# JADGardner/neusky

Measured on AMD Instinct MI355X. Metric: train rays/sec on NeRF-OSR lk2 @1024 rays x 96 samples, higher is better.
Workload: dtype f32 in memory; forward products: fp16 hi + residual split, 3 x v_mfma_f32_32x32x16_f16 per product on power-of-two pre-scaled operands, one fp32 accumulator (~2^-22): FiLM-SIREN chains and the SDF / albedo field alike; backward products: the same fp16 split on per-row / per-matrix pre-scaled gradien; 1 GPU; full NeuSky train step (BASELINE configs[2]): 1024 rays/GPU x 96 samples, proposal 256+96, 512 illumination directions (256 upper-hemisphere DDF queries/ray), illumination decoder = this project's FiLM-SIREN H = 128 (RENI-shaped: latent 100x3; the reference's configured Attention decoder is absent from its tree), hash L16 F2 T2^19 x2, 256-wide MLPs; fwd + losses + bwd + all-reduce + 5 Adam groups; rays_per_gpu=1024, samples_per_ray=96, illumination_directions=512, parallelism=ray-sharded dp1, launcher=self-spawned, launch=HIP graph replay (1 graph/step + all-reduce + 5 Adam launches)

## Files before the change

include/neusky_hip.h:

```cpp
#ifndef NEUSKY_HIP_H
#define NEUSKY_HIP_H

#include <stdint.h>

#ifdef __cplusplus
extern "C" {
#endif

typedef void* nsky_stream_t;

const char* nsky_last_error(void);
int nsky_abi_version(void);

enum {
  NSKY_EPI_NONE = 0,
  NSKY_EPI_RELU = 1,
  NSKY_EPI_LEAKY = 2,
  NSKY_EPI_SIGMOID = 3,
  NSKY_EPI_SOFTPLUS = 4,
  NSKY_EPI_FILM = 5,
  NSKY_EPI_MUL_AUX = 6,
  NSKY_EPI_BWD_RELU = 7,
  NSKY_EPI_BWD_LEAKY = 8,
  NSKY_EPI_BWD_FILM = 9,
// ... 44 lines not shown
  const float* mo_w; const float* mo_b; int32_t mo_ld;
  const float* film_w[NSKY_FILM_MAX_LAYERS]; const float* film_b[NSKY_FILM_MAX_LAYERS]; int32_t film_ld[NSKY_FILM_MAX_LAYERS];
  const float* out_w; const float* out_b; int32_t out_ld;
} nsky_film_net;
int nsky_film_stream_layout(const nsky_film_net* net, int32_t direction, int64_t* stream_bytes, int32_t* n_tiles);
int nsky_film_pack(const nsky_film_net* net, int32_t direction, void* stream_buf, float* table, nsky_stream_t stream);
int nsky_film_chain_fwd(const nsky_film_net* net, const void* stream_buf, const float* table, const float* cond,
                        int32_t ldcond, const float* x, int32_t ldx, int32_t M, float* const* h_save, float* const* z_save,
                        float* const* y_save, float* res, int32_t ldres, nsky_stream_t stream);
int nsky_film_chain_bwd_film(const nsky_film_net* net, const void* stream_buf, const float* table, int32_t M, const float* d_res,
                             int32_t ldres, const float* h_last, const float* const* z_save, float* const* dz_save, float* dfp,
                             float* dfp_rowmax, float* gmax, float* d_x, int32_t ldx, nsky_stream_t stream);
int nsky_film_chain_bwd_map(const nsky_film_net* net, const void* stream_buf, const float* table, int32_t M, const float* dfp,
                            const float* dfp_rowmax, const float* const* h_save, float* const* dpre_save, float* d_cond,
                            int32_t ldcond, float* gmax, nsky_stream_t stream);
typedef struct {
  int32_t in_dim, hidden;
  const float* w0; int32_t ld0; const float* b0;
  const float* w1; int32_t ld1; const float* b1;
  const float* w2; const float* b2;
  float beta;
} nsky_sdf_net;
int nsky_sdf_stream_layout(const nsky_sdf_net* net, int32_t direction, int64_t* stream_bytes, int32_t* n_tiles);
int nsky_sdf_pack(const nsky_sdf_net* net, int32_t direction, void* stream_buf, float* table, nsky_stream_t stream);
int nsky_sdf_chain_fwd(const nsky_sdf_net* net, const void* stream_buf, const float* table, const float* E, int32_t ldE, int32_t M,
                       float* a0_save, float* a1_save, float* sdf, nsky_stream_t stream);
int nsky_sdf_chain_bwd(const nsky_sdf_net* net, const void* stream_buf, const float* table, int32_t M, const float* g_sdf,
                       const float* a0_save, const float* a1_save, float* dz1, float* dz0, float* dE, int32_t ldE, float* dw2,
                       float* db2, float* gmax, nsky_stream_t stream);

// ... 346 lines not shown
```

neusky_amd/csrc/film_chain.hip:

```cpp
#include "chain.h"

namespace {

constexpr int FWD_FRAG_BUFFERS = 3;


struct Layout {
  int NT, Gc, Gx, Gh;
  long base_map, base_film0, base_film, base_head, total_groups;
  int n_tiles;
};

__host__ __device__ inline Layout fwd_layout(const nsky_film_net& n) {
  Layout L;
  L.NT = n.hidden / 32;
  L.Gc = groups_of(n.cond_dim);
  L.Gx = groups_of(n.x_dim);
  L.Gh = groups_of(n.hidden);
  L.base_map = (long)L.NT * L.Gc;
  L.base_film0 = L.base_map + (long)(n.n_map - 1) * L.NT * L.Gh;
  L.base_film = L.base_film0 + (long)L.NT * (2 * L.Gh + L.Gx);
  L.base_head = L.base_film + (long)(n.n_film - 1) * L.NT * 3 * L.Gh;
  L.total_groups = L.base_head + L.Gh;
  L.n_tiles = n.n_map * L.NT + n.n_film * L.NT * 3 + 1;
// ... 125 lines not shown
}



struct FwdArgs {
  nsky_film_net net;
  const unsigned char* stream;
  const float* table;
  const float* cond; int ldcond;
  const float* x; int ldx;
  int M;
  float* h_save[MAXL];
  float* z_save[MAXL];
  float* y_save[MAXL];
  float* res; int ldres;
};


template <int H, int KSC, bool KEEP_Y = true>
__global__ __launch_bounds__(256, 1) void film_fwd_kernel(const FwdArgs a) {
  constexpr int NT = H / 32, KS = H / 16;
  __shared__ __attribute__((aligned(16))) unsigned char smem[RING_BYTES + (BIAS_FLOATS + SCALE_FLOATS) * 4];
  float* bl = reinterpret_cast<float*>(smem + RING_BYTES);
  const nsky_film_net& net = a.net;
  const int tid = threadIdx.x, lane = tid & 63;
  const int wave = __builtin_amdgcn_readfirstlane(tid >> 6);
  const int c = lane & 31, h = lane >> 5;
  float* sl = bl + BIAS_FLOATS;
  NSKY_STAGE_TABLE((BIAS_FLOATS + SCALE_FLOATS) / 4, 256, a.table, bl, tid);
  __syncthreads();
  WStream ws;
  ws_open<4, false, RING_GROUPS, true>(ws, a.stream, smem, wave, lane);

  const long rt = (long)blockIdx.x * 4 + wave;
// ... 7 lines not shown
  f16x8 hh[KS], hl[KS];
  float h_inv;
  {
    f16x8 ch[KSC], cl[KSC];
    const int ksc = ksteps_of(net.cond_dim);
    const float c_inv = load_planes<KSC>(a.cond + rowc * a.ldcond, (net.cond_dim + 3) & ~3, ksc, h, ch, cl);
    float hn[NT][16];
    float m = 0.0f;
#pragma unroll
    for (int t = 0; t < NT; ++t) {
      f32x16 acc;
#pragma unroll
      for (int r = 0; r < 16; ++r) acc[r] = 0.0f;
      product_dyn<KSC>(ws, ksc, ch, cl, acc);
      const float inv = c_inv * sl[tile++];
#pragma unroll
      for (int g = 0; g < 4; ++g) {
        const float4 b = *reinterpret_cast<const float4*>(bl + 32 * t + 8 * g + 4 * h);
        const float bb[4] = {b.x, b.y, b.z, b.w};
#pragma unroll
        for (int q = 0; q < 4; ++q) {
          const float v = fmaf(acc[4 * g + q], inv, bb[q]);
          const float o = v > 0.0f ? v : 0.2f * v;
          hn[t][4 * g + q] = o;
          m = fmaxf(m, fabsf(o));
        }
      }
      if (a.h_save[0] && wave_live) store_tile_nt(a.h_save[0] + (rt * NT + t) * 1024, lane, hn[t]);
    }
    const float s = row_scale(m, h_inv);
#pragma unroll
    for (int t = 0; t < NT; ++t)
#pragma unroll
      for (int u = 0; u < 2; ++u) {
        float x8[8];
#pragma unroll
        for (int j = 0; j < 8; ++j) x8[j] = hn[t][8 * u + j] * s;
        split8(x8, hh[2 * t + u], hl[2 * t + u]);
      }
  }
  for (int l = 1; l < n_map; ++l) {
    float hn[NT][16];
    float m = 0.0f;
    const float* bias = bl + l * H;
#pragma unroll
    for (int t = 0; t < NT; ++t) {
      f32x16 acc;
#pragma unroll
      for (int r = 0; r < 16; ++r) acc[r] = 0.0f;
      product<KS, 4, false, RING_GROUPS, FWD_FRAG_BUFFERS>(ws, hh, hl, acc);
      const float inv = h_inv * sl[tile++];
#pragma unroll
      for (int g = 0; g < 4; ++g) {
        const float4 b = *reinterpret_cast<const float4*>(bias + 32 * t + 8 * g + 4 * h);
        const float bb[4] = {b.x, b.y, b.z, b.w};
#pragma unroll
        for (int q = 0; q < 4; ++q) {
          const float v = fmaf(acc[4 * g + q], inv, bb[q]);
          const float o = v > 0.0f ? v : 0.2f * v;
          hn[t][4 * g + q] = o;
          m = fmaxf(m, fabsf(o));
        }
      }
      if (a.h_save[l] && wave_live) store_tile_nt(a.h_save[l] + (rt * NT + t) * 1024, lane, hn[t]);
    }
    const float s = row_scale(m, h_inv);
#pragma unroll
    for (int t = 0; t < NT; ++t)
#pragma unroll
      for (int u = 0; u < 2; ++u) {
        float x8[8];
#pragma unroll
        for (int j = 0; j < 8; ++j) x8[j] = hn[t][8 * u + j] * s;
        split8(x8, hh[2 * t + u], hl[2 * t + u]);
      }
  }
  f16x8 xh[1], xl[1];
  const float x_inv = load_planes<1>(a.x + rowc * a.ldx, (net.x_dim + 3) & ~3, 1, h, xh, xl);
  f16x8 yh[KS], yl[KS];
// ... 309 lines not shown
  ws_close();
}

struct BwdMapArgs {
  nsky_film_net net;
  const unsigned char* stream;
  const float* table;
  int M;
  const float* dfp;
  const float* dfp_rowmax;
  const float* h_save[MAXL];
  float* dpre_save[MAXL];
  float* d_cond; int ldcond;
  float* gmax;
  int full_wgs, tail_wgs, tail_k;
};

template <int H, bool ACTIVE, bool KEEP>
__device__ __forceinline__ void film_bwd_map_tile(const BwdMapArgs& a, WStream& ws, const float* sl, long rt, int lane) {
  constexpr int NT = H / 32, KS = H / 16, PW = 2;
  constexpr bool REGS = !KEEP && H <= 128;
  float dreg[REGS ? NT : 1][16];
  const nsky_film_net& net = a.net;
  const int c = lane & 31, h = lane >> 5;
  const long row = rt * 32 + c;
  const bool live = ACTIVE && row < a.M;
  const int nkb = 2 * net.n_film * H / 64, ntot = 2 * net.n_film * NT;
  float f_inv = 1.0f, f_scale = 1.0f;
  if (ACTIVE) f_scale = row_scale(a.dfp_rowmax[rt * 32 + c], f_inv);
  int tile = 0;
  const float* fblk = a.dfp + rt * ntot * 1024;
  const int top = net.n_map - 1;
  float m = 0.0f;
// ... 95 lines not shown
          float x8[8];
#pragma unroll
          for (int j = 0; j < 8; ++j) x8[j] = dv[8 * v + j] * s;
          split8(x8, ph[2 * u + v], pl[2 * u + v]);
        }
      }
      asm volatile("s_waitcnt vmcnt(0)" ::: "memory");
    }
    m = 0.0f;
    if (l > 0) {
      for (int u = 0; u < NT; ++u) {
        f32x16 acc;
        prod<KS, PW>(ws, ACTIVE, ph, pl, acc);
        if (ACTIVE) {
          const float inv = d_inv * sl[tile];
          float hv[16], dv[16];
          load_tile(a.h_save[l - 1] + (rt * NT + u) * 1024, lane, hv);
#pragma unroll
          for (int r = 0; r < 16; ++r) {
            const float g = acc[r] * inv;
            dv[r] = hv[r] > 0.0f ? g : 0.2f * g;
            m = fmaxf(m, fabsf(dv[r]));
          }
          if constexpr (REGS) {
#pragma unroll
            for (int uu = 0; uu < NT; ++uu)
              if (u == uu) {
#pragma unroll
                for (int r = 0; r < 16; ++r) dreg[uu][r] = dv[r];
              }
          } else {
            store_tile(a.dpre_save[l - 1] + (rt * NT + u) * 1024, lane, dv);
          }
          asm volatile("s_waitcnt vmcnt(0)" ::: "memory");
        }
        ++tile;
      }
// ... 5 lines not shown
        if (ACTIVE && a.d_cond && live) {
          const float inv = d_inv * sl[tile];
#pragma unroll
          for (int g = 0; g < 4; ++g) {
            const int fo = 32 * u + 8 * g + 4 * h;
            if (fo < a.ldcond)
              stg4(a.d_cond + row * a.ldcond + fo, make_float4(acc[4 * g] * inv, acc[4 * g + 1] * inv, acc[4 * g + 2] * inv, acc[4 * g + 3] * inv));
          }
        }
        ++tile;
      }
    }
  }
}

template <int H, bool KEEP = true>
__global__ __launch_bounds__(512, 2) void film_bwd_map_kernel(const BwdMapArgs a) {
  constexpr int PW = 2;
  __shared__ __attribute__((aligned(16))) unsigned char smem[RING_BYTES + SCALE_FLOATS * 4];
  float* sl = reinterpret_cast<float*>(smem + RING_BYTES);
  const int tid = threadIdx.x, lane = tid & 63;
  const int wave = __builtin_amdgcn_readfirstlane(tid >> 6);
  for (int i = tid; i < SCALE_FLOATS; i += 512) sl[i] = a.table[BIAS_FLOATS + i];
  __syncthreads();
  WStream ws;
  ws_open<PW>(ws, a.stream, smem, wave, lane);
  const long n_tiles = (a.M + 31) / 32;
  const long rt = tail_tile(a.full_wgs, a.tail_wgs, a.tail_k, n_tiles, wave);
  if (rt >= 0 && rt < n_tiles) film_bwd_map_tile<H, true, KEEP>(a, ws, sl, rt, lane);
  else film_bwd_map_tile<H, false, KEEP>(a, ws, sl, 0, lane);
  ws_close();
}

int check_net(const nsky_film_net* n, const char* who) {
  NSKY_CHECK_ARG(n, "%s: null network", who);
  NSKY_CHECK_ARG(n->hidden == 128 || n->hidden == 256, "%s: hidden width %d (128 or 256)", who, n->hidden);
  NSKY_CHECK_ARG(n->n_map >= 1 && n->n_map <= MAXL && n->n_film >= 1 && n->n_film <= MAXL, "%s: layer counts %d / %d", who, n->n_map, n->n_film);
  NSKY_CHECK_ARG(n->cond_dim >= 1 && n->cond_dim <= PACK_KMAX && n->x_dim >= 1 && n->x_dim <= 16 && n->out_dim >= 1 && n->out_dim <= 4,
                 "%s: cond_dim %d (<= %d), x_dim %d (<= 16), out_dim %d (<= 4)", who, n->cond_dim, PACK_KMAX, n->x_dim, n->out_dim);
  const int nb = n->n_map * n->hidden + 3 * n->n_film * n->hidden + 32;
  NSKY_CHECK_ARG(nb <= BIAS_FLOATS, "%s: %d bias values exceed the LDS table (%d)", who, nb, BIAS_FLOATS);
  NSKY_CHECK_ARG(fwd_layout(*n).n_tiles <= SCALE_FLOATS, "%s: %d weight tiles exceed the LDS scale table (%d)", who, fwd_layout(*n).n_tiles, SCALE_FLOATS);
  for (int l = 0; l < n->n_map; ++l) NSKY_CHECK_ARG(n->map_w[l] && n->map_ld[l] >= (l == 0 ? n->cond_dim : n->hidden), "%s: mapping layer %d", who, l);
  for (int l = 0; l < n->n_film; ++l) NSKY_CHECK_ARG(n->film_w[l] && n->film_ld[l] >= (l == 0 ? n->x_dim : n->hidden), "%s: FiLM layer %d", who, l);
  NSKY_CHECK_ARG(n->mo_w && n->mo_ld >= n->hidden && n->out_w && n->out_ld >= n->hidden, "%s: head weights", who);
// ... 15 lines not shown
}

extern "C" int nsky_film_pack(const nsky_film_net* net, int32_t direction, void* stream_buf, float* table, nsky_stream_t stream) {
  if (int rc = check_net(net, "nsky_film_pack")) return rc;
  NSKY_CHECK_ARG(direction >= 0 && direction <= 2 && stream_buf && table && ((uintptr_t)stream_buf % 16) == 0 && ((uintptr_t)table % 16) == 0, "nsky_film_pack: bad arguments");
  long groups;
  int tiles;
  dir_layout(*net, direction, groups, tiles);
  NSKY_CHECK_ARG(tiles <= SCALE_FLOATS, "nsky_film_pack: %d weight tiles exceed the scale table (%d)", tiles, SCALE_FLOATS);
  if (direction != 0) NSKY_CHECK_ARG(net->hidden % 128 == 0, "nsky_film_pack: backward streams need hidden %% 128 == 0");
  hipLaunchKernelGGL(film_pack_kernel, dim3(tiles + 1), dim3(256), 0, (hipStream_t)stream, *net, direction, (unsigned char*)stream_buf, table);
  NSKY_CHECK_LAUNCH("nsky_film_pack");
  return NSKY_OK;
}

extern "C" int nsky_film_chain_fwd(const nsky_film_net* net, const void* stream_buf, const float* table, const float* cond,
                                   int32_t ldcond, const float* x, int32_t ldx, int32_t M, float* const* h_save, float* const* z_save,
                                   float* const* y_save, float* res, int32_t ldres, nsky_stream_t stream) {
  if (int rc = check_net(net, "nsky_film_chain_fwd")) return rc;
  NSKY_CHECK_ARG(stream_buf && table && cond && x && res && M > 0, "nsky_film_chain_fwd: null operand / empty batch");
  NSKY_CHECK_ARG(ldcond % 4 == 0 && ldcond >= ((net->cond_dim + 3) & ~3) && ldx % 4 == 0 && ldx >= ((net->x_dim + 3) & ~3) && ldres >= 4 && ldres % 4 == 0,
                 "nsky_film_chain_fwd: leading dimensions (cond %d, x %d, res %d) must be multiples of 4 covering the padded widths", ldcond, ldx, ldres);
  NSKY_CHECK_ARG(((uintptr_t)cond % 16) == 0 && ((uintptr_t)x % 16) == 0 && ((uintptr_t)res % 16) == 0 && ((uintptr_t)stream_buf % 16) == 0 && ((uintptr_t)table % 16) == 0,
                 "nsky_film_chain_fwd: operands must be 16-byte aligned");
  FwdArgs a;
  a.net = *net;
  a.stream = (const unsigned char*)stream_buf; a.table = table;
  a.cond = cond; a.ldcond = ldcond; a.x = x; a.ldx = ldx; a.M = M; a.res = res; a.ldres = ldres;
  for (int l = 0; l < MAXL; ++l) {
    a.h_save[l] = (h_save && l < net->n_map) ? h_save[l] : nullptr;
    a.z_save[l] = (z_save && l < net->n_film) ? z_save[l] : nullptr;
    a.y_save[l] = (y_save && l < net->n_film) ? y_save[l] : nullptr;
  }
  const bool keep_y = a.y_save[0] != nullptr;
  NSKY_CHECK_ARG(keep_y || net->hidden == 128, "nsky_film_chain_fwd: NULL y_save needs hidden 128 (hidden %d: pass two ping-pong buffers)", net->hidden);
  for (int l = 0; l < net->n_film; ++l)
    NSKY_CHECK_ARG((a.y_save[l] != nullptr) == keep_y && ((uintptr_t)a.y_save[l] % 16) == 0, "nsky_film_chain_fwd: y_save[%d] missing / unaligned", l);
  const dim3 grid(ceil_div(M, 128));
  const int ksc = ksteps_of(net->cond_dim);
#define NSKY_FILM_FWD(HH, KK, KEEP) hipLaunchKernelGGL((film_fwd_kernel<HH, KK, KEEP>), grid, dim3(256), 0, (hipStream_t)stream, a)
  if (net->hidden == 256) { if (ksc <= 4) NSKY_FILM_FWD(256, 4, true); else NSKY_FILM_FWD(256, 20, true); }
  else if (keep_y) { if (ksc <= 4) NSKY_FILM_FWD(128, 4, true); else NSKY_FILM_FWD(128, 20, true); }
  else { if (ksc <= 4) NSKY_FILM_FWD(128, 4, false); else NSKY_FILM_FWD(128, 20, false); }
#undef NSKY_FILM_FWD
  NSKY_CHECK_LAUNCH("nsky_film_chain_fwd");
  return NSKY_OK;
}


extern "C" int nsky_film_chain_bwd_film(const nsky_film_net* net, const void* stream_buf, const float* table, int32_t M, const float* d_res,
                                        int32_t ldres, const float* h_last, const float* const* z_save, float* const* dz_save, float* dfp,
                                        float* dfp_rowmax, float* gmax, float* d_x, int32_t ldx, nsky_stream_t stream) {
  if (int rc = check_net(net, "nsky_film_chain_bwd_film")) return rc;
  NSKY_CHECK_ARG(stream_buf && table && d_res && h_last && z_save && dfp && dfp_rowmax && gmax && M > 0, "nsky_film_chain_bwd_film: null operand / empty batch");
  NSKY_CHECK_ARG(ldres >= 4 && ldres % 4 == 0 && ((uintptr_t)d_res % 16) == 0 && ((uintptr_t)h_last % 16) == 0 && ((uintptr_t)dfp % 16) == 0 &&
                     ((uintptr_t)stream_buf % 16) == 0 && ((uintptr_t)table % 16) == 0, "nsky_film_chain_bwd_film: alignment / ldres");
  NSKY_CHECK_ARG(net->hidden % 128 == 0, "nsky_film_chain_bwd_film: hidden %% 128");
  BwdFilmArgs a;
  a.net = *net; a.stream = (const unsigned char*)stream_buf; a.table = table; a.M = M; a.d_res = d_res; a.ldres = ldres; a.h_last = h_last;
  a.dfp = dfp; a.dfp_rowmax = dfp_rowmax; a.gmax = gmax; a.d_x = d_x; a.ldx = ldx;
  if (d_x) NSKY_CHECK_ARG(ldx % 4 == 0 && ldx >= ((net->x_dim + 3) & ~3) && ldx <= 16 && ((uintptr_t)d_x % 16) == 0, "nsky_film_chain_bwd_film: d_x layout (ldx %d)", ldx);
// ... 2 lines not shown
    a.dz_save[l] = (dz_save && l < net->n_film) ? dz_save[l] : nullptr;
  }
  const bool keep = a.dz_save[0] != nullptr;
  for (int l = 0; l < net->n_film; ++l)
    NSKY_CHECK_ARG(a.z_save[l] && (a.dz_save[l] != nullptr) == keep && ((uintptr_t)a.z_save[l] % 16) == 0 && ((uintptr_t)a.dz_save[l] % 16) == 0, "nsky_film_chain_bwd_film: z_save / dz_save[%d]", l);
  a.full_wgs = a.tail_wgs = a.tail_k = 0;
  const dim3 grid(ceil_div(ceil_div(M, 32), 4));
#define NSKY_FILM_BWD4(HH, KEEP) hipLaunchKernelGGL((film_bwd4_kernel<HH, KEEP>), grid, dim3(256), 0, (hipStream_t)stream, a)
  if (net->hidden == 256) { if (keep) NSKY_FILM_BWD4(256, true); else NSKY_FILM_BWD4(256, false); }
  else { if (keep) NSKY_FILM_BWD4(128, true); else NSKY_FILM_BWD4(128, false); }
#undef NSKY_FILM_BWD4
  NSKY_CHECK_LAUNCH("nsky_film_chain_bwd_film");
  return NSKY_OK;
}

extern "C" int nsky_film_chain_bwd_map(const nsky_film_net* net, const void* stream_buf, const float* table, int32_t M, const float* dfp,
                                       const float* dfp_rowmax, const float* const* h_save, float* const* dpre_save, float* d_cond,
                                       int32_t ldcond, float* gmax, nsky_stream_t stream) {
  if (int rc = check_net(net, "nsky_film_chain_bwd_map")) return rc;
  NSKY_CHECK_ARG(stream_buf && table && dfp && dfp_rowmax && h_save && gmax && M > 0, "nsky_film_chain_bwd_map: null operand / empty batch");
  NSKY_CHECK_ARG(((uintptr_t)dfp % 16) == 0 && ((uintptr_t)stream_buf % 16) == 0 && ((uintptr_t)table % 16) == 0, "nsky_film_chain_bwd_map: alignment");
  if (d_cond) NSKY_CHECK_ARG(ldcond % 4 == 0 && ldcond >= ((net->cond_dim + 3) & ~3) && ((uintptr_t)d_cond % 16) == 0, "nsky_film_chain_bwd_map: d_cond layout");
  NSKY_CHECK_ARG(net->hidden % 128 == 0, "nsky_film_chain_bwd_map: hidden %% 128");
  BwdMapArgs a;
  a.net = *net; a.stream = (const unsigned char*)stream_buf; a.table = table; a.M = M; a.dfp = dfp; a.dfp_rowmax = dfp_rowmax;
  a.d_cond = d_cond; a.ldcond = ldcond; a.gmax = gmax;
  for (int l = 0; l < MAXL; ++l) {
    a.h_save[l] = l < net->n_map ? h_save[l] : nullptr;
    a.dpre_save[l] = (dpre_save && l < net->n_map) ? dpre_save[l] : nullptr;
  }
  const bool regs = a.dpre_save[0] == nullptr;
  const bool keep = !regs && !(net->n_map > 1 && a.dpre_save[1] == a.dpre_save[0]);
  NSKY_CHECK_ARG(!regs || net->hidden == 128, "nsky_film_chain_bwd_map: NULL dpre_save needs hidden 128 (hidden %d: pass one shared buffer)", net->hidden);
  for (int l = 0; l < net->n_map; ++l)
    NSKY_CHECK_ARG(a.h_save[l] && (a.dpre_save[l] == nullptr) == regs && (keep || a.dpre_save[l] == a.dpre_save[0]) && ((uintptr_t)a.h_save[l] % 16) == 0 &&
                       ((uintptr_t)a.dpre_save[l] % 16) == 0, "nsky_film_chain_bwd_map: h_save / dpre_save[%d]", l);
  const TailPlan tp = tail_plan(ceil_div(M, 32), device_cus());
  a.full_wgs = tp.full_wgs; a.tail_wgs = tp.tail_wgs; a.tail_k = tp.tail_k;
  const dim3 grid(tp.full_wgs + tp.tail_wgs);
#define NSKY_FILM_BWD_MAP(HH, KEEP) hipLaunchKernelGGL((film_bwd_map_kernel<HH, KEEP>), grid, dim3(512), 0, (hipStream_t)stream, a)
  if (net->hidden == 256) { if (keep) NSKY_FILM_BWD_MAP(256, true); else NSKY_FILM_BWD_MAP(256, false); }
  else { if (keep) NSKY_FILM_BWD_MAP(128, true); else NSKY_FILM_BWD_MAP(128, false); }
#undef NSKY_FILM_BWD_MAP
  NSKY_CHECK_LAUNCH("nsky_film_chain_bwd_map");
  return NSKY_OK;
}
```

neusky_amd/hip.py:

```python
from __future__ import annotations

import ctypes as C
import os

import torch

_HERE = os.path.dirname(os.path.abspath(__file__))
LIB_PATH = os.path.join(_HERE, "libneusky_hip.so")


class NeuSkyHipError(RuntimeError):
    pass


if not os.path.exists(LIB_PATH):
    raise ImportError(
        f"{LIB_PATH} not found: build the HIP extension first (python -c 'import __graft_entry__ as g; g.build()'). "
        "neusky_amd has no CPU/PyTorch fallback."
    )
_lib = C.CDLL(LIB_PATH)

EPI_NONE, EPI_RELU, EPI_LEAKY, EPI_SIGMOID, EPI_SOFTPLUS, EPI_FILM, EPI_MUL_AUX = 0, 1, 2, 3, 4, 5, 6
EPI_BWD_RELU, EPI_BWD_LEAKY, EPI_BWD_FILM, EPI_EXP = 7, 8, 9, 10
PREC_F32, PREC_BF16X2, PREC_BF16X3, PREC_F16X2 = 0, 2, 3, 4
# ... 611 lines not shown


class FilmNet(C.Structure):
    _fields_ = [("hidden", C.c_int32), ("n_map", C.c_int32), ("n_film", C.c_int32),
                ("cond_dim", C.c_int32), ("x_dim", C.c_int32), ("out_dim", C.c_int32),
                ("map_w", C.c_void_p * FILM_MAX_LAYERS), ("map_b", C.c_void_p * FILM_MAX_LAYERS), ("map_ld", C.c_int32 * FILM_MAX_LAYERS),
                ("mo_w", C.c_void_p), ("mo_b", C.c_void_p), ("mo_ld", C.c_int32),
                ("film_w", C.c_void_p * FILM_MAX_LAYERS), ("film_b", C.c_void_p * FILM_MAX_LAYERS), ("film_ld", C.c_int32 * FILM_MAX_LAYERS),
                ("out_w", C.c_void_p), ("out_b", C.c_void_p), ("out_ld", C.c_int32)]


_film_layout = _sig("nsky_film_stream_layout", C.POINTER(FilmNet), C.c_int32, C.POINTER(C.c_int64), C.POINTER(C.c_int32))
_film_pack = _sig("nsky_film_pack", C.POINTER(FilmNet), C.c_int32, C.c_void_p, C.c_void_p, C.c_void_p)
_film_fwd = _sig("nsky_film_chain_fwd", C.POINTER(FilmNet), C.c_void_p, C.c_void_p, C.c_void_p, C.c_int32, C.c_void_p, C.c_int32, C.c_int32,
                 C.c_void_p, C.c_void_p, C.c_void_p, C.c_void_p, C.c_int32, C.c_void_p)


_film_bwd_film = _sig("nsky_film_chain_bwd_film", C.POINTER(FilmNet), C.c_void_p, C.c_void_p, C.c_int32, C.c_void_p, C.c_int32, C.c_void_p,
                      C.c_void_p, C.c_void_p, C.c_void_p, C.c_void_p, C.c_void_p, C.c_void_p, C.c_int32, C.c_void_p)
_film_bwd_map = _sig("nsky_film_chain_bwd_map", C.POINTER(FilmNet), C.c_void_p, C.c_void_p, C.c_int32, C.c_void_p, C.c_void_p, C.c_void_p,
                     C.c_void_p, C.c_void_p, C.c_int32, C.c_void_p, C.c_void_p)


_wgrad_native = _sig("nsky_wgrad_native", C.c_void_p, C.c_int32, C.c_void_p, C.c_int32, C.c_int32, C.c_void_p, C.c_int32, C.c_void_p,
                     C.c_void_p, C.c_float, C.c_void_p)


class WgradProblem(C.Structure):
    _fields_ = [("dZ", C.c_void_p), ("nnt_a", C.c_int32), ("X", C.c_void_p), ("nnt_b", C.c_int32), ("dW", C.c_void_p), ("ldw", C.c_int32),
                ("db", C.c_void_p), ("a_scale_max", C.c_void_p), ("b_scale", C.c_float),
                ("lda", C.c_int32), ("ldb", C.c_int32), ("width_a", C.c_int32), ("width_b", C.c_int32), ("bias_rows", C.c_int32),
                ("bias_row_mod", C.c_int32), ("b_scale_max", C.c_void_p)]


WGRAD_MAX_PROBLEMS = 16
_wgrad_native_batch = _sig("nsky_wgrad_native_batch", C.POINTER(WgradProblem), C.c_int32, C.c_int32, C.c_void_p)
# ... 304 lines not shown
def quad_native_to_rows(buf, N: int, width: int):
    return film_native_to_rows(buf, 4 * N, width).reshape(N, 4, width).permute(1, 0, 2)


def _ptr_array(ts, n):
    arr = (C.c_void_p * FILM_MAX_LAYERS)()
    for i in range(n):
        arr[i] = None if ts is None or ts[i] is None else ts[i].data_ptr()
    return arr


def film_keepless(hidden: int) -> str:
    return "registers" if hidden == 128 else "buffers"


def film_chain_fwd(net: FilmNet, stream_buf, scales, cond, x, M, h_save, z_save, y_save, res):
    check(_film_fwd(C.byref(net), ptr(stream_buf), ptr(scales), ptr(cond), ld(cond), ptr(x), ld(x), M,
                    _ptr_array(h_save, net.n_map), _ptr_array(z_save, net.n_film), _ptr_array(y_save, net.n_film), ptr(res), ld(res),
                    stream_ptr()), "nsky_film_chain_fwd")
    return res


def film_rows(M: int) -> int:
    return (M + 31) // 32 * 32


def film_native_to_rows(buf, M: int, width: int):
    R = film_rows(M) // 32
    return buf.reshape(R, width // 32, 4, 2, 32, 4).permute(0, 4, 1, 2, 3, 5).reshape(R * 32, width)[:M]


def film_rows_to_native(x, width: int):
    M = x.shape[0]
    R = film_rows(M) // 32
    full = x.new_zeros(R * 32, width)
    full[:M] = x[:, :width]
    return full.reshape(R, 32, width // 32, 4, 2, 4).permute(0, 2, 3, 4, 1, 5).contiguous().reshape(R * 32, width)


def film_chain_bwd_film(net: FilmNet, stream_buf, table, M, d_res, h_last, z_save, dz_save, dfp, dfp_rowmax, gmax, d_x=None):
    check(_film_bwd_film(C.byref(net), ptr(stream_buf), ptr(table), M, ptr(d_res), ld(d_res), ptr(h_last), _ptr_array(z_save, net.n_film),
                         _ptr_array(dz_save, net.n_film), ptr(dfp), ptr(dfp_rowmax), ptr(gmax), ptr(d_x), ld(d_x) if d_x is not None else 0,
                         stream_ptr()), "nsky_film_chain_bwd_film")


def film_chain_bwd_map(net: FilmNet, stream_buf, table, M, dfp, dfp_rowmax, h_save, dpre_save, d_cond, gmax):
    check(_film_bwd_map(C.byref(net), ptr(stream_buf), ptr(table), M, ptr(dfp), ptr(dfp_rowmax), _ptr_array(h_save, net.n_map),
                        _ptr_array(dpre_save, net.n_map), ptr(d_cond), ld(d_cond) if d_cond is not None else 0, ptr(gmax), stream_ptr()),
          "nsky_film_chain_bwd_map")


MC_TILE = 256
_mc_count = _sig("nsky_mc_count", C.c_void_p, C.c_int64, C.c_int64, C.c_int64, C.c_float, C.c_void_p, C.c_void_p)
_mc_vertices = _sig("nsky_mc_vertices", C.c_void_p, C.c_int64, C.c_int64, C.c_int64, C.c_float, C.c_float, C.c_float, C.c_float,
                    C.c_float, C.c_float, C.c_float, C.c_void_p, C.c_void_p, C.c_void_p, C.c_void_p, C.c_void_p)
_mc_faces = _sig("nsky_mc_faces", C.c_void_p, C.c_int64, C.c_int64, C.c_int64, C.c_float, C.c_void_p, C.c_void_p, C.c_void_p,
                 C.c_void_p, C.c_void_p)


def mc_count(volume, level: float, tile_counts):
    nx, ny, nz = volume.shape
    check(_mc_count(ptr(volume), nx, ny, nz, level, ptr(tile_counts), stream_ptr()), "nsky_mc_count")


# ... 322 lines not shown
```

neusky_amd/ops.py:

```python
from __future__ import annotations

from typing import List, Optional, Sequence

import torch
import torch.nn.functional as F

from . import hip


_POLICIES = ("f32", "splith")
_FWD = {"splith": hip.PREC_F16X2}
_POLICY = "splith"
FWD_PRECISION = _FWD.get(_POLICY, hip.PREC_F32)
BWD_PRECISION = hip.PREC_F32


def set_precision_policy(policy: str) -> None:
    global FWD_PRECISION, _POLICY
    if policy not in _POLICIES:
        raise ValueError(policy)
    _POLICY = policy
    FWD_PRECISION = _FWD.get(policy, hip.PREC_F32)


# ... 589 lines not shown


def _film_stream(wb, n_map, n_film, direction=0):
    key = (wb[0].data_ptr(), wb[0]._version, wb[-2].data_ptr(), n_map, n_film, direction)

    def pack():
        mw, mb, mwo, mbo, fw, fb, ow, ob, _ = _film_unpack(wb, n_map, n_film)
        net = hip.film_net(mw[0].shape[1], fw[0].shape[1], ow.shape[0], mw, mb, mwo, mbo, fw, fb, ow, ob)
        nbytes, _ = hip.film_stream_layout(net, direction)
        stream, table = _stream_buffers(("film", stable_id(wb[0]), n_map, n_film, direction), nbytes, hip.FILM_TABLE_FLOATS, wb[0].device)
        hip.film_pack(net, stream, table, direction)
        return net, stream, table
    return _prepared(_FILM_STREAMS, key, list(wb), pack)


class FilmChainFn(torch.autograd.Function):

    @staticmethod
    def forward(ctx, x, cond, n_map, n_film, train_weights, need_dcond, *wb):
        M = x.shape[0]
        dev = x.device
        mw, _, _, _, fw, _, ow, _, _ = _film_unpack(wb, n_map, n_film)
        H, Hm, n_out_p = fw[0].shape[0], mw[0].shape[0], ow.shape[0]
        save = any(ctx.needs_input_grad)
        train_w = train_weights and any(ctx.needs_input_grad[6:])
        keep_y = save and train_w
        net, stream, scales = _film_stream(wb, n_map, n_film)
        Mp = hip.film_rows(M)
        if keep_y:
            ys = [torch.empty(Mp, H, device=dev) for _ in range(n_film)]
        elif save and hip.film_keepless(H) == "registers":
            ys = None
        else:
            pp = [torch.empty(Mp, H, device=dev) for _ in range(min(2, n_film))]
            ys = [pp[i % len(pp)] for i in range(n_film)]
        hs = [torch.empty(Mp, Hm, device=dev) for _ in range(n_map)] if save else None
        zs = [torch.empty(Mp, H, device=dev) for _ in range(n_film)] if save else None
        res = torch.empty(M, n_out_p, device=dev)
        hip.film_chain_fwd(net, stream, scales, cond, x, M, hs, zs, ys, res)
        if not save:
            return res
        ctx.save_for_backward(x, cond, *hs, *(ys if keep_y else []), *zs, *wb)
        ctx.cfg = (n_map, n_film, train_w, need_dcond, M, H, Hm, x.requires_grad)
        ctx.sinks = [_sink_param(w) for w in wb]
        ctx.pad_sinks = [_sink_param(w, "pad") for w in wb]
        return res

    @staticmethod
    def backward(ctx, d_res):
        n_map, n_film, train_w, need_dcond, M, H, Hm, need_dx = ctx.cfg
        sv = ctx.saved_tensors
        x, cond = sv[0], sv[1]
        hs = list(sv[2:2 + n_map])
        n_ys = n_film if train_w else 0
        ys = list(sv[2 + n_map:2 + n_map + n_ys])
        zs = list(sv[2 + n_map + n_ys:2 + n_map + n_ys + n_film])
        wb = sv[2 + n_map + n_ys + n_film:]
        mw, mb, mwo, mbo, fw, fb, ow, ob, o = _film_unpack(wb, n_map, n_film)
        dev = x.device
        Mp = hip.film_rows(M)
        d_res = d_res.contiguous()
        net1, s1, t1 = _film_stream(wb, n_map, n_film, 1)
        net2, s2, t2 = _film_stream(wb, n_map, n_film, 2)
        dzs = [torch.empty(Mp, H, device=dev) for _ in range(n_film)] if train_w else None
        dfp = torch.empty(Mp, 2 * n_film * H, device=dev)
        rowmax = torch.empty(Mp, device=dev)
        gmax = zeros(n_film + 1 + n_map, device=dev)
        d_x = torch.empty(M, ld(x), device=dev) if need_dx else None
        hip.film_chain_bwd_film(net1, s1, t1, M, d_res, hs[-1], zs, dzs, dfp, rowmax, gmax[:n_film + 1], d_x)
        d_cond = torch.empty(M, ld(cond), device=dev) if need_dcond else None
        want_map = need_dcond or train_w
        if train_w:
            dpres = [torch.empty(Mp, Hm, device=dev) for _ in range(n_map)]
        elif want_map and hip.film_keepless(Hm) == "buffers":
            dpres = [torch.empty(Mp, Hm, device=dev)] * n_map
        else:
            dpres = None
        if want_map:
            hip.film_chain_bwd_map(net2, s2, t2, M, dfp, rowmax, hs, dpres, d_cond, gmax[n_film + 1:])
        if not train_w:
            return (d_x, d_cond, None, None, None, None, *[None] * len(wb))
        grads, sunk = _carve_grads(wb, _sink_grads(ctx.sinks, from_first_pass=True))
        nt, ntm = H // 32, Hm // 32
        native = []

        def wgrad(dZ, X, n_out, k_in, like, bias_like, iw, a_nt, b_nt, smax, x_scale=64.0):
            if a_nt > 0 and b_nt > 0 and a_nt % 4 == 0 and b_nt % 4 == 0 and smax is not None:
                native.append(hip.wgrad_problem(dZ, a_nt, X, b_nt, M, grads[iw], grads[iw + 1], smax, x_scale))
            elif a_nt == 0 and b_nt > 0 and n_out <= 4 and dZ.dim() == 2 and dZ.shape[1] == 4 and dZ.is_contiguous():
                hip.native_weighted_colsum(X, b_nt, M, grads[iw], grads[iw + 1], w4=dZ, n_out=n_out)
            else:
                grad_weight(dZ, X, M, n_out, k_in, like, bias_like, acc=(grads[iw], grads[iw + 1]), a_native_nt=a_nt, b_native_nt=b_nt,
                            a_scale_max=smax)

# ... 1120 lines not shown
```

Measured before the change: 53280 rays/s.

## Save leaky-ReLU sign bitmaps instead of full activations for FiLM mapping backward

The FiLM mapping-network forward pass now records one bit per activation (pre-activation sign) into a 16-bit-per-lane bitmap. The backward mapping kernel uses that bitmap to pick the leaky-ReLU slope instead of reloading full fp32 hidden-state tiles. When weights are not trained, only the last mapping layer's activations are kept in fp32, which cuts activation memory and backward read traffic. With weight training on, the fp32 saves are still written, so the extra bitmap writes add a little cost on that path. The change also adds template variants and new C entry points.

```diff
diff --git a/include/neusky_hip.h b/include/neusky_hip.h
--- a/include/neusky_hip.h
+++ b/include/neusky_hip.h
@@ -82,6 +82,12 @@
 int nsky_film_chain_bwd_map(const nsky_film_net* net, const void* stream_buf, const float* table, int32_t M, const float* dfp,
                             const float* dfp_rowmax, const float* const* h_save, float* const* dpre_save, float* d_cond,
                             int32_t ldcond, float* gmax, nsky_stream_t stream);
+int nsky_film_chain_fwd_signs(const nsky_film_net* net, const void* stream_buf, const float* table, const float* cond,
+                              int32_t ldcond, const float* x, int32_t ldx, int32_t M, float* const* h_save, float* const* z_save,
+                              float* const* y_save, float* res, int32_t ldres, uint16_t* const* sign_save, nsky_stream_t stream);
+int nsky_film_chain_bwd_map_signs(const nsky_film_net* net, const void* stream_buf, const float* table, int32_t M, const float* dfp,
+                                  const float* dfp_rowmax, const float* const* h_save, float* const* dpre_save, float* d_cond,
+                                  int32_t ldcond, float* gmax, const uint16_t* const* sign_save, nsky_stream_t stream);
 typedef struct {
   int32_t in_dim, hidden;
   const float* w0; int32_t ld0; const float* b0;
diff --git a/neusky_amd/csrc/film_chain.hip b/neusky_amd/csrc/film_chain.hip
--- a/neusky_amd/csrc/film_chain.hip
+++ b/neusky_amd/csrc/film_chain.hip
@@ -163,10 +163,11 @@
   float* z_save[MAXL];
   float* y_save[MAXL];
   float* res; int ldres;
+  unsigned short* sign_save[MAXL];
 };
 
 
-template <int H, int KSC, bool KEEP_Y = true>
+template <int H, int KSC, bool KEEP_Y = true, bool SIGNS = false>
 __global__ __launch_bounds__(256, 1) void film_fwd_kernel(const FwdArgs a) {
   constexpr int NT = H / 32, KS = H / 16;
   __shared__ __attribute__((aligned(16))) unsigned char smem[RING_BYTES + (BIAS_FLOATS + SCALE_FLOATS) * 4];
@@ -204,6 +205,7 @@
       for (int r = 0; r < 16; ++r) acc[r] = 0.0f;
       product_dyn<KSC>(ws, ksc, ch, cl, acc);
       const float inv = c_inv * sl[tile++];
+      unsigned bits = 0;
 #pragma unroll
       for (int g = 0; g < 4; ++g) {
         const float4 b = *reinterpret_cast<const float4*>(bl + 32 * t + 8 * g + 4 * h);
@@ -212,11 +214,14 @@
         for (int q = 0; q < 4; ++q) {
           const float v = fmaf(acc[4 * g + q], inv, bb[q]);
           const float o = v > 0.0f ? v : 0.2f * v;
+          if constexpr (SIGNS) bits |= (v > 0.0f ? 1u : 0u) << (4 * g + q);
           hn[t][4 * g + q] = o;
           m = fmaxf(m, fabsf(o));
         }
       }
       if (a.h_save[0] && wave_live) store_tile_nt(a.h_save[0] + (rt * NT + t) * 1024, lane, hn[t]);
+      if constexpr (SIGNS)
+        if (a.sign_save[0] && wave_live) a.sign_save[0][(rt * NT + t) * 64 + lane] = (unsigned short)bits;
     }
     const float s = row_scale(m, h_inv);
 #pragma unroll
@@ -240,6 +245,7 @@
       for (int r = 0; r < 16; ++r) acc[r] = 0.0f;
       product<KS, 4, false, RING_GROUPS, FWD_FRAG_BUFFERS>(ws, hh, hl, acc);
       const float inv = h_inv * sl[tile++];
+      unsigned bits = 0;
 #pragma unroll
       for (int g = 0; g < 4; ++g) {
         const float4 b = *reinterpret_cast<const float4*>(bias + 32 * t + 8 * g + 4 * h);
@@ -248,11 +254,14 @@
         for (int q = 0; q < 4; ++q) {
           const float v = fmaf(acc[4 * g + q], inv, bb[q]);
           const float o = v > 0.0f ? v : 0.2f * v;
+          if constexpr (SIGNS) bits |= (v > 0.0f ? 1u : 0u) << (4 * g + q);
           hn[t][4 * g + q] = o;
           m = fmaxf(m, fabsf(o));
         }
       }
       if (a.h_save[l] && wave_live) store_tile_nt(a.h_save[l] + (rt * NT + t) * 1024, lane, hn[t]);
+      if constexpr (SIGNS)
+        if (a.sign_save[l] && wave_live) a.sign_save[l][(rt * NT + t) * 64 + lane] = (unsigned short)bits;
     }
     const float s = row_scale(m, h_inv);
 #pragma unroll
@@ -592,9 +601,12 @@
   float* d_cond; int ldcond;
   float* gmax;
   int full_wgs, tail_wgs, tail_k;
+  const unsigned short* sign_save[MAXL];
 };
 
-template <int H, bool ACTIVE, bool KEEP>
+__device__ __forceinline__ unsigned sign_word(const unsigned short* signs, long tile_index, int lane) { return signs[tile_index * 64 + lane]; }
+
+template <int H, bool ACTIVE, bool KEEP, bool SIGNS>
 __device__ __forceinline__ void film_bwd_map_tile(const BwdMapArgs& a, WStream& ws, const float* sl, long rt, int lane) {
   constexpr int NT = H / 32, KS = H / 16, PW = 2;
   constexpr bool REGS = !KEEP && H <= 128;
@@ -720,13 +732,24 @@
         prod<KS, PW>(ws, ACTIVE, ph, pl, acc);
         if (ACTIVE) {
           const float inv = d_inv * sl[tile];
-          float hv[16], dv[16];
-          load_tile(a.h_save[l - 1] + (rt * NT + u) * 1024, lane, hv);
-#pragma unroll
-          for (int r = 0; r < 16; ++r) {
-            const float g = acc[r] * inv;
-            dv[r] = hv[r] > 0.0f ? g : 0.2f * g;
-            m = fmaxf(m, fabsf(dv[r]));
+          float dv[16];
+          if constexpr (SIGNS) {
+            const unsigned sb = sign_word(a.sign_save[l - 1], rt * NT + u, lane);
+#pragma unroll
+            for (int r = 0; r < 16; ++r) {
+              const float g = acc[r] * inv;
+              dv[r] = (sb >> r) & 1u ? g : 0.2f * g;
+              m = fmaxf(m, fabsf(dv[r]));
+            }
+          } else {
+            float hv[16];
+            load_tile(a.h_save[l - 1] + (rt * NT + u) * 1024, lane, hv);
+#pragma unroll
+            for (int r = 0; r < 16; ++r) {
+              const float g = acc[r] * inv;
+              dv[r] = hv[r] > 0.0f ? g : 0.2f * g;
+              m = fmaxf(m, fabsf(dv[r]));
+            }
           }
           if constexpr (REGS) {
 #pragma unroll
@@ -762,7 +785,7 @@
   }
 }
 
-template <int H, bool KEEP = true>
+template <int H, bool KEEP = true, bool SIGNS = false>
 __global__ __launch_bounds__(512, 2) void film_bwd_map_kernel(const BwdMapArgs a) {
   constexpr int PW = 2;
   __shared__ __attribute__((aligned(16))) unsigned char smem[RING_BYTES + SCALE_FLOATS * 4];
@@ -775,8 +798,8 @@
   ws_open<PW>(ws, a.stream, smem, wave, lane);
   const long n_tiles = (a.M + 31) / 32;
   const long rt = tail_tile(a.full_wgs, a.tail_wgs, a.tail_k, n_tiles, wave);
-  if (rt >= 0 && rt < n_tiles) film_bwd_map_tile<H, true, KEEP>(a, ws, sl, rt, lane);
-  else film_bwd_map_tile<H, false, KEEP>(a, ws, sl, 0, lane);
+  if (rt >= 0 && rt < n_tiles) film_bwd_map_tile<H, true, KEEP, SIGNS>(a, ws, sl, rt, lane);
+  else film_bwd_map_tile<H, false, KEEP, SIGNS>(a, ws, sl, 0, lane);
   ws_close();
 }
 
@@ -822,9 +845,10 @@
   return NSKY_OK;
 }
 
-extern "C" int nsky_film_chain_fwd(const nsky_film_net* net, const void* stream_buf, const float* table, const float* cond,
-                                   int32_t ldcond, const float* x, int32_t ldx, int32_t M, float* const* h_save, float* const* z_save,
-                                   float* const* y_save, float* res, int32_t ldres, nsky_stream_t stream) {
+namespace {
+int film_fwd_launch(const nsky_film_net* net, const void* stream_buf, const float* table, const float* cond, int32_t ldcond, const float* x,
+                    int32_t ldx, int32_t M, float* const* h_save, float* const* z_save, float* const* y_save, float* res, int32_t ldres,
+                    uint16_t* const* sign_save, nsky_stream_t stream) {
   if (int rc = check_net(net, "nsky_film_chain_fwd")) return rc;
   NSKY_CHECK_ARG(stream_buf && table && cond && x && res && M > 0, "nsky_film_chain_fwd: null operand / empty batch");
   NSKY_CHECK_ARG(ldcond % 4 == 0 && ldcond >= ((net->cond_dim + 3) & ~3) && ldx % 4 == 0 && ldx >= ((net->x_dim + 3) & ~3) && ldres >= 4 && ldres % 4 == 0,
@@ -839,6 +863,8 @@
     a.h_save[l] = (h_save && l < net->n_map) ? h_save[l] : nullptr;
     a.z_save[l] = (z_save && l < net->n_film) ? z_save[l] : nullptr;
     a.y_save[l] = (y_save && l < net->n_film) ? y_save[l] : nullptr;
+    a.sign_save[l] = (sign_save && l < net->n_map) ? sign_save[l] : nullptr;
+    NSKY_CHECK_ARG(((uintptr_t)a.sign_save[l] % 16) == 0 && ((uintptr_t)a.h_save[l] % 16) == 0, "nsky_film_chain_fwd: h_save / sign_save[%d] unaligned", l);
   }
   const bool keep_y = a.y_save[0] != nullptr;
   NSKY_CHECK_ARG(keep_y || net->hidden == 128, "nsky_film_chain_fwd: NULL y_save needs hidden 128 (hidden %d: pass two ping-pong buffers)", net->hidden);
@@ -846,13 +872,31 @@
     NSKY_CHECK_ARG((a.y_save[l] != nullptr) == keep_y && ((uintptr_t)a.y_save[l] % 16) == 0, "nsky_film_chain_fwd: y_save[%d] missing / unaligned", l);
   const dim3 grid(ceil_div(M, 128));
   const int ksc = ksteps_of(net->cond_dim);
-#define NSKY_FILM_FWD(HH, KK, KEEP) hipLaunchKernelGGL((film_fwd_kernel<HH, KK, KEEP>), grid, dim3(256), 0, (hipStream_t)stream, a)
+#define NSKY_FILM_FWD(HH, KK, KEEP)                                                                                        \
+  do {                                                                                                                    \
+    if (sign_save) hipLaunchKernelGGL((film_fwd_kernel<HH, KK, KEEP, true>), grid, dim3(256), 0, (hipStream_t)stream, a); \
+    else hipLaunchKernelGGL((film_fwd_kernel<HH, KK, KEEP, false>), grid, dim3(256), 0, (hipStream_t)stream, a);          \
+  } while (0)
   if (net->hidden == 256) { if (ksc <= 4) NSKY_FILM_FWD(256, 4, true); else NSKY_FILM_FWD(256, 20, true); }
   else if (keep_y) { if (ksc <= 4) NSKY_FILM_FWD(128, 4, true); else NSKY_FILM_FWD(128, 20, true); }
   else { if (ksc <= 4) NSKY_FILM_FWD(128, 4, false); else NSKY_FILM_FWD(128, 20, false); }
 #undef NSKY_FILM_FWD
   NSKY_CHECK_LAUNCH("nsky_film_chain_fwd");
   return NSKY_OK;
+}
+}
+
+extern "C" int nsky_film_chain_fwd(const nsky_film_net* net, const void* stream_buf, const float* table, const float* cond,
+                                   int32_t ldcond, const float* x, int32_t ldx, int32_t M, float* const* h_save, float* const* z_save,
+                                   float* const* y_save, float* res, int32_t ldres, nsky_stream_t stream) {
+  return film_fwd_launch(net, stream_buf, table, cond, ldcond, x, ldx, M, h_save, z_save, y_save, res, ldres, nullptr, stream);
+}
+
+extern "C" int nsky_film_chain_fwd_signs(const nsky_film_net* net, const void* stream_buf, const float* table, const float* cond,
+                                         int32_t ldcond, const float* x, int32_t ldx, int32_t M, float* const* h_save, float* const* z_save,
+                                         float* const* y_save, float* res, int32_t ldres, uint16_t* const* sign_save, nsky_stream_t stream) {
+  NSKY_CHECK_ARG(sign_save, "nsky_film_chain_fwd_signs: null sign_save");
+  return film_fwd_launch(net, stream_buf, table, cond, ldcond, x, ldx, M, h_save, z_save, y_save, res, ldres, sign_save, stream);
 }
 
 
@@ -885,9 +929,10 @@
   return NSKY_OK;
 }
 
-extern "C" int nsky_film_chain_bwd_map(const nsky_film_net* net, const void* stream_buf, const float* table, int32_t M, const float* dfp,
-                                       const float* dfp_rowmax, const float* const* h_save, float* const* dpre_save, float* d_cond,
-                                       int32_t ldcond, float* gmax, nsky_stream_t stream) {
+namespace {
+int film_bwd_map_launch(const nsky_film_net* net, const void* stream_buf, const float* table, int32_t M, const float* dfp,
+                        const float* dfp_rowmax, const float* const* h_save, float* const* dpre_save, float* d_cond, int32_t ldcond,
+                        float* gmax, const uint16_t* const* sign_save, nsky_stream_t stream) {
   if (int rc = check_net(net, "nsky_film_chain_bwd_map")) return rc;
   NSKY_CHECK_ARG(stream_buf && table && dfp && dfp_rowmax && h_save && gmax && M > 0, "nsky_film_chain_bwd_map: null operand / empty batch");
   NSKY_CHECK_ARG(((uintptr_t)dfp % 16) == 0 && ((uintptr_t)stream_buf % 16) == 0 && ((uintptr_t)table % 16) == 0, "nsky_film_chain_bwd_map: alignment");
@@ -897,22 +942,45 @@
   a.net = *net; a.stream = (const unsigned char*)stream_buf; a.table = table; a.M = M; a.dfp = dfp; a.dfp_rowmax = dfp_rowmax;
   a.d_cond = d_cond; a.ldcond = ldcond; a.gmax = gmax;
   for (int l = 0; l < MAXL; ++l) {
-    a.h_save[l] = l < net->n_map ? h_save[l] : nullptr;
+    a.h_save[l] = (h_save && l < net->n_map) ? h_save[l] : nullptr;
     a.dpre_save[l] = (dpre_save && l < net->n_map) ? dpre_save[l] : nullptr;
+    a.sign_save[l] = (sign_save && l < net->n_map) ? sign_save[l] : nullptr;
   }
   const bool regs = a.dpre_save[0] == nullptr;
   const bool keep = !regs && !(net->n_map > 1 && a.dpre_save[1] == a.dpre_save[0]);
   NSKY_CHECK_ARG(!regs || net->hidden == 128, "nsky_film_chain_bwd_map: NULL dpre_save needs hidden 128 (hidden %d: pass one shared buffer)", net->hidden);
+  for (int l = 0; l < net->n_map; ++l) {
+    const bool from_bitmap = sign_save && l < net->n_map - 1;
+    NSKY_CHECK_ARG(from_bitmap ? a.sign_save[l] != nullptr : a.h_save[l] != nullptr, "nsky_film_chain_bwd_map: layer %d has no %s", l, from_bitmap ? "sign bitmap" : "h_save");
+  }
   for (int l = 0; l < net->n_map; ++l)
-    NSKY_CHECK_ARG(a.h_save[l] && (a.dpre_save[l] == nullptr) == regs && (keep || a.dpre_save[l] == a.dpre_save[0]) && ((uintptr_t)a.h_save[l] % 16) == 0 &&
+    NSKY_CHECK_ARG(((uintptr_t)a.sign_save[l] % 16) == 0 && (a.dpre_save[l] == nullptr) == regs && (keep || a.dpre_save[l] == a.dpre_save[0]) && ((uintptr_t)a.h_save[l] % 16) == 0 &&
                        ((uintptr_t)a.dpre_save[l] % 16) == 0, "nsky_film_chain_bwd_map: h_save / dpre_save[%d]", l);
   const TailPlan tp = tail_plan(ceil_div(M, 32), device_cus());
   a.full_wgs = tp.full_wgs; a.tail_wgs = tp.tail_wgs; a.tail_k = tp.tail_k;
   const dim3 grid(tp.full_wgs + tp.tail_wgs);
-#define NSKY_FILM_BWD_MAP(HH, KEEP) hipLaunchKernelGGL((film_bwd_map_kernel<HH, KEEP>), grid, dim3(512), 0, (hipStream_t)stream, a)
+#define NSKY_FILM_BWD_MAP(HH, KEEP)                                                                                        \
+  do {                                                                                                                    \
+    if (sign_save) hipLaunchKernelGGL((film_bwd_map_kernel<HH, KEEP, true>), grid, dim3(512), 0, (hipStream_t)stream, a); \
+    else hipLaunchKernelGGL((film_bwd_map_kernel<HH, KEEP, false>), grid, dim3(512), 0, (hipStream_t)stream, a);          \
+  } while (0)
   if (net->hidden == 256) { if (keep) NSKY_FILM_BWD_MAP(256, true); else NSKY_FILM_BWD_MAP(256, false); }
   else { if (keep) NSKY_FILM_BWD_MAP(128, true); else NSKY_FILM_BWD_MAP(128, false); }
 #undef NSKY_FILM_BWD_MAP
   NSKY_CHECK_LAUNCH("nsky_film_chain_bwd_map");
   return NSKY_OK;
 }
+}
+
+extern "C" int nsky_film_chain_bwd_map(const nsky_film_net* net, const void* stream_buf, const float* table, int32_t M, const float* dfp,
+                                       const float* dfp_rowmax, const float* const* h_save, float* const* dpre_save, float* d_cond,
+                                       int32_t ldcond, float* gmax, nsky_stream_t stream) {
+  return film_bwd_map_launch(net, stream_buf, table, M, dfp, dfp_rowmax, h_save, dpre_save, d_cond, ldcond, gmax, nullptr, stream);
+}
+
+extern "C" int nsky_film_chain_bwd_map_signs(const nsky_film_net* net, const void* stream_buf, const float* table, int32_t M, const float* dfp,
+                                             const float* dfp_rowmax, const float* const* h_save, float* const* dpre_save, float* d_cond,
+                                             int32_t ldcond, float* gmax, const uint16_t* const* sign_save, nsky_stream_t stream) {
+  NSKY_CHECK_ARG(sign_save, "nsky_film_chain_bwd_map_signs: null sign_save");
+  return film_bwd_map_launch(net, stream_buf, table, M, dfp, dfp_rowmax, h_save, dpre_save, d_cond, ldcond, gmax, sign_save, stream);
+}
diff --git a/neusky_amd/hip.py b/neusky_amd/hip.py
--- a/neusky_amd/hip.py
+++ b/neusky_amd/hip.py
@@ -649,12 +649,16 @@
 _film_pack = _sig("nsky_film_pack", C.POINTER(FilmNet), C.c_int32, C.c_void_p, C.c_void_p, C.c_void_p)
 _film_fwd = _sig("nsky_film_chain_fwd", C.POINTER(FilmNet), C.c_void_p, C.c_void_p, C.c_void_p, C.c_int32, C.c_void_p, C.c_int32, C.c_int32,
                  C.c_void_p, C.c_void_p, C.c_void_p, C.c_void_p, C.c_int32, C.c_void_p)
+_film_fwd_signs = _sig("nsky_film_chain_fwd_signs", C.POINTER(FilmNet), C.c_void_p, C.c_void_p, C.c_void_p, C.c_int32, C.c_void_p, C.c_int32,
+                       C.c_int32, C.c_void_p, C.c_void_p, C.c_void_p, C.c_void_p, C.c_int32, C.c_void_p, C.c_void_p)
 
 
 _film_bwd_film = _sig("nsky_film_chain_bwd_film", C.POINTER(FilmNet), C.c_void_p, C.c_void_p, C.c_int32, C.c_void_p, C.c_int32, C.c_void_p,
                       C.c_void_p, C.c_void_p, C.c_void_p, C.c_void_p, C.c_void_p, C.c_void_p, C.c_int32, C.c_void_p)
 _film_bwd_map = _sig("nsky_film_chain_bwd_map", C.POINTER(FilmNet), C.c_void_p, C.c_void_p, C.c_int32, C.c_void_p, C.c_void_p, C.c_void_p,
                      C.c_void_p, C.c_void_p, C.c_int32, C.c_void_p, C.c_void_p)
+_film_bwd_map_signs = _sig("nsky_film_chain_bwd_map_signs", C.POINTER(FilmNet), C.c_void_p, C.c_void_p, C.c_int32, C.c_void_p, C.c_void_p,
+                           C.c_void_p, C.c_void_p, C.c_void_p, C.c_int32, C.c_void_p, C.c_void_p, C.c_void_p)
 
 
 _wgrad_native = _sig("nsky_wgrad_native", C.c_void_p, C.c_int32, C.c_void_p, C.c_int32, C.c_int32, C.c_void_p, C.c_int32, C.c_void_p,
@@ -989,11 +993,34 @@
     return "registers" if hidden == 128 else "buffers"
 
 
-def film_chain_fwd(net: FilmNet, stream_buf, scales, cond, x, M, h_save, z_save, y_save, res):
-    check(_film_fwd(C.byref(net), ptr(stream_buf), ptr(scales), ptr(cond), ld(cond), ptr(x), ld(x), M,
-                    _ptr_array(h_save, net.n_map), _ptr_array(z_save, net.n_film), _ptr_array(y_save, net.n_film), ptr(res), ld(res),
-                    stream_ptr()), "nsky_film_chain_fwd")
+def film_sign_words(M: int, hidden: int) -> int:
+    return film_rows(M) * hidden // 16
+
+
+def film_signs_to_rows(signs, M: int, hidden: int):
+    R, NT = film_rows(M) // 32, hidden // 32
+    w = signs.reshape(R, NT, 2, 32).to(torch.int32) & 0xFFFF
+    bits = (w.unsqueeze(-1) >> torch.arange(16, device=signs.device, dtype=torch.int32)) & 1
+    return bits.reshape(R, NT, 2, 32, 4, 4).permute(0, 3, 1, 4, 2, 5).reshape(R * 32, hidden)[:M].bool()
+
+
+def film_chain_fwd(net: FilmNet, stream_buf, scales, cond, x, M, h_save, z_save, y_save, res, sign_save=None):
+    if sign_save is None:
+        check(_film_fwd(C.byref(net), ptr(stream_buf), ptr(scales), ptr(cond), ld(cond), ptr(x), ld(x), M,
+                        _ptr_array(h_save, net.n_map), _ptr_array(z_save, net.n_film), _ptr_array(y_save, net.n_film), ptr(res), ld(res),
+                        stream_ptr()), "nsky_film_chain_fwd")
+    else:
+        _check_signs(sign_save, net, M)
+        check(_film_fwd_signs(C.byref(net), ptr(stream_buf), ptr(scales), ptr(cond), ld(cond), ptr(x), ld(x), M,
+                              _ptr_array(h_save, net.n_map), _ptr_array(z_save, net.n_film), _ptr_array(y_save, net.n_film), ptr(res), ld(res),
+                              _ptr_array(sign_save, net.n_map), stream_ptr()), "nsky_film_chain_fwd_signs")
     return res
+
+
+def _check_signs(sign_save, net, M):
+    for s in sign_save[:net.n_map]:
+        if s is not None and (s.dtype != torch.int16 or s.numel() < film_sign_words(M, net.hidden) or not s.is_contiguous()):
+            raise ValueError(f"sign bitmap: contiguous int16 tensor of at least {film_sign_words(M, net.hidden)} elements, got {s.dtype} x {s.numel()}")
 
 
 def film_rows(M: int) -> int:
@@ -1019,10 +1046,16 @@
                          stream_ptr()), "nsky_film_chain_bwd_film")
 
 
-def film_chain_bwd_map(net: FilmNet, stream_buf, table, M, dfp, dfp_rowmax, h_save, dpre_save, d_cond, gmax):
-    check(_film_bwd_map(C.byref(net), ptr(stream_buf), ptr(table), M, ptr(dfp), ptr(dfp_rowmax), _ptr_array(h_save, net.n_map),
-                        _ptr_array(dpre_save, net.n_map), ptr(d_cond), ld(d_cond) if d_cond is not None else 0, ptr(gmax), stream_ptr()),
-          "nsky_film_chain_bwd_map")
+def film_chain_bwd_map(net: FilmNet, stream_buf, table, M, dfp, dfp_rowmax, h_save, dpre_save, d_cond, gmax, sign_save=None):
+    if sign_save is None:
+        check(_film_bwd_map(C.byref(net), ptr(stream_buf), ptr(table), M, ptr(dfp), ptr(dfp_rowmax), _ptr_array(h_save, net.n_map),
+                            _ptr_array(dpre_save, net.n_map), ptr(d_cond), ld(d_cond) if d_cond is not None else 0, ptr(gmax), stream_ptr()),
+              "nsky_film_chain_bwd_map")
+    else:
+        _check_signs(sign_save, net, M)
+        check(_film_bwd_map_signs(C.byref(net), ptr(stream_buf), ptr(table), M, ptr(dfp), ptr(dfp_rowmax), _ptr_array(h_save, net.n_map),
+                                  _ptr_array(dpre_save, net.n_map), ptr(d_cond), ld(d_cond) if d_cond is not None else 0, ptr(gmax),
+                                  _ptr_array(sign_save, net.n_map), stream_ptr()), "nsky_film_chain_bwd_map_signs")
 
 
 MC_TILE = 256
diff --git a/neusky_amd/ops.py b/neusky_amd/ops.py
--- a/neusky_amd/ops.py
+++ b/neusky_amd/ops.py
@@ -627,6 +627,9 @@
     return _prepared(_FILM_STREAMS, key, list(wb), pack)
 
 
+FILM_SIGN_BITMAPS = True
+
+
 class FilmChainFn(torch.autograd.Function):
 
     @staticmethod
@@ -647,13 +650,18 @@
         else:
             pp = [torch.empty(Mp, H, device=dev) for _ in range(min(2, n_film))]
             ys = [pp[i % len(pp)] for i in range(n_film)]
-        hs = [torch.empty(Mp, Hm, device=dev) for _ in range(n_map)] if save else None
+        signs_on = save and FILM_SIGN_BITMAPS
+        n_hs = n_map if (train_w or not signs_on) else 1
+        hs = [None] * (n_map - n_hs) + [torch.empty(Mp, Hm, device=dev) for _ in range(n_hs)] if save else None
+        n_signs = n_map - 1 if signs_on else 0
+        signs = [torch.empty(hip.film_sign_words(M, Hm), dtype=torch.int16, device=dev) for _ in range(n_signs)] + [None] * (n_map - n_signs)
         zs = [torch.empty(Mp, H, device=dev) for _ in range(n_film)] if save else None
         res = torch.empty(M, n_out_p, device=dev)
-        hip.film_chain_fwd(net, stream, scales, cond, x, M, hs, zs, ys, res)
+        hip.film_chain_fwd(net, stream, scales, cond, x, M, hs, zs, ys, res, signs if n_signs else None)
         if not save:
             return res
-        ctx.save_for_backward(x, cond, *hs, *(ys if keep_y else []), *zs, *wb)
+        ctx.save_for_backward(x, cond, *hs[n_map - n_hs:], *signs[:n_signs], *(ys if keep_y else []), *zs, *wb)
+        ctx.film_saved = (n_hs, n_signs)
         ctx.cfg = (n_map, n_film, train_w, need_dcond, M, H, Hm, x.requires_grad)
         ctx.sinks = [_sink_param(w) for w in wb]
         ctx.pad_sinks = [_sink_param(w, "pad") for w in wb]
@@ -664,11 +672,14 @@
         n_map, n_film, train_w, need_dcond, M, H, Hm, need_dx = ctx.cfg
         sv = ctx.saved_tensors
         x, cond = sv[0], sv[1]
-        hs = list(sv[2:2 + n_map])
+        n_hs, n_signs = ctx.film_saved
+        hs = [None] * (n_map - n_hs) + list(sv[2:2 + n_hs])
+        signs = (list(sv[2 + n_hs:2 + n_hs + n_signs]) + [None] * (n_map - n_signs)) if n_signs else None
+        o_ys = 2 + n_hs + n_signs
         n_ys = n_film if train_w else 0
-        ys = list(sv[2 + n_map:2 + n_map + n_ys])
-        zs = list(sv[2 + n_map + n_ys:2 + n_map + n_ys + n_film])
-        wb = sv[2 + n_map + n_ys + n_film:]
+        ys = list(sv[o_ys:o_ys + n_ys])
+        zs = list(sv[o_ys + n_ys:o_ys + n_ys + n_film])
+        wb = sv[o_ys + n_ys + n_film:]
         mw, mb, mwo, mbo, fw, fb, ow, ob, o = _film_unpack(wb, n_map, n_film)
         dev = x.device
         Mp = hip.film_rows(M)
@@ -690,7 +701,7 @@
         else:
             dpres = None
         if want_map:
-            hip.film_chain_bwd_map(net2, s2, t2, M, dfp, rowmax, hs, dpres, d_cond, gmax[n_film + 1:])
+            hip.film_chain_bwd_map(net2, s2, t2, M, dfp, rowmax, hs, dpres, d_cond, gmax[n_film + 1:], signs)
         if not train_w:
             return (d_x, d_cond, None, None, None, None, *[None] * len(wb))
         grads, sunk = _carve_grads(wb, _sink_grads(ctx.sinks, from_first_pass=True))
```

After: 53550 rays/s, median of 6. No clear change (+0.5%).
